# david-strejc/fei

Hardware: AMD Instinct MI355X
Metric: agent tok/s (llama3-8b local decode, 1 agent/GPU) (higher is better)
Workload: dtype bf16; 1 GPU; model=llama3-8b, global_batch=1, seq_len=512, parallelism=dp1 (1 agent per GPU, weak scaling), hip_graph=True, stream_engine=False

## Files before the change

fei_amd/ops/__init__.py:

```python

from __future__ import annotations

import ctypes
import math
import os
from typing import Optional, Tuple

import torch

from fei_amd.ops import reference as ref

_LIB: Optional[ctypes.CDLL] = None
_LIB_ERR: Optional[str] = None
_LIB_PATH = os.path.join(os.path.dirname(os.path.abspath(__file__)),
                         "libfei_kernels.so")

_c = ctypes
_vp, _i, _f, _u64, _l = _c.c_void_p, _c.c_int, _c.c_float, _c.c_ulonglong, _c.c_long


def _try_load() -> None:
    global _LIB, _LIB_ERR
    if _LIB is not None or _LIB_ERR is not None:
        return
    try:
        lib = ctypes.CDLL(_LIB_PATH)
    except OSError as e:
        _LIB_ERR = str(e)
        return
    lib.fei_rmsnorm.argtypes = [_vp, _vp, _vp, _i, _i, _f, _vp]
    lib.fei_add_rmsnorm.argtypes = [_vp, _vp, _vp, _vp, _i, _i, _f, _vp]
    lib.fei_rope_kv_decode.argtypes = [_vp, _vp, _vp, _vp, _vp, _vp, _vp,
                                       _i, _i, _i, _i, _i, _l, _l, _vp]
    lib.fei_rope_kv_prefill.argtypes = [_vp, _vp, _vp, _vp, _vp, _vp, _vp,
                                        _i, _i, _i, _i, _i, _i, _l, _l, _vp]
    lib.fei_attn_decode.argtypes = [_vp, _vp, _vp, _vp, _vp, _vp,
                                    _i, _i, _i, _i, _i, _i, _f, _l,
                                    _vp, _vp, _vp, _l, _vp, _vp, _i, _vp]
    lib.fei_attn_decode_combine.argtypes = [_vp, _vp, _vp, _i, _i, _i, _i, _vp]
    lib.fei_swiglu.argtypes = [_vp, _vp, _l, _i, _vp]
    lib.fei_sample.argtypes = [_vp, _vp, _vp, _vp, _vp, _i, _i, _i, _f, _u64,
                               _i, _vp]
    lib.fei_advance.argtypes = [_vp, _vp, _i, _i, _vp]
    lib.fei_attn_prefill.argtypes = [_vp, _vp, _vp, _vp, _vp, _vp,
                                     _i, _i, _i, _i, _i, _i, _f, _i, _l, _vp]
    lib.fei_mfma_probe.argtypes = [_vp, _vp, _vp, _vp]
    lib.fei_gemv.argtypes = [_vp, _vp, _vp, _i, _i, _i, _i, _vp]
    lib.fei_gemm_m8.argtypes = [_vp, _vp, _vp, _i, _i, _i, _i, _vp]
    lib.fei_attn_decode_fused.argtypes = [_vp, _vp, _vp, _vp, _vp, _vp, _vp,
                                          _vp, _i, _i, _i, _i, _i, _f,
                                          _l, _l, _vp]
    lib.fei_sample_onepass.argtypes = [_vp, _vp, _vp, _vp, _i, _i, _f, _u64,
                                       _i, _vp]
    lib.fei_sample_shard.argtypes = [_vp, _vp, _vp, _i, _i, _i, _f, _u64, _vp]
    lib.fei_sample_filtered.argtypes = [_vp, _vp, _vp, _vp, _vp, _i, _i, _i,
                                        _f, _f, _u64, _i, _vp]
    lib.fei_sample_filtered_rows.argtypes = [_vp, _vp, _vp, _vp, _vp, _vp,
                                             _vp, _vp, _i, _i, _vp]
    lib.fei_sample_filtered_rows.restype = _i
    lib.fei_rope_kv8_decode.argtypes = [_vp, _vp, _vp, _vp, _vp, _vp, _vp,
                                        _vp, _vp, _i, _i, _i, _i, _i, _l, _l,
                                        _vp]
    lib.fei_rope_kv8_prefill.argtypes = [_vp, _vp, _vp, _vp, _vp, _vp, _vp,
                                         _vp, _vp, _i, _i, _i, _i, _i, _i,
                                         _l, _l, _vp]
    lib.fei_attn_decode_kv8.argtypes = [_vp, _vp, _vp, _vp, _vp, _vp, _vp,
                                        _vp, _i, _i, _i, _i, _i, _i, _f, _l,
                                        _vp, _vp, _vp, _l, _vp]
    lib.fei_attn_decode_kv8.restype = _i
    lib.fei_attn_prefill_kv8.argtypes = [_vp, _vp, _vp, _vp, _vp, _vp, _vp,
                                         _i, _i, _i, _i, _i, _i, _f, _l, _vp]
    lib.fei_attn_prefill_kv8.restype = _i
    lib.fei_stream_layer_check.argtypes = [_i, _i, _i, _i, _i]
    lib.fei_stream_layer_check.restype = _i
    lib.fei_stream_layer.argtypes = [_vp, _vp, _vp, _vp, _vp, _vp, _vp, _vp,
                                     _vp, _vp, _vp, _vp, _vp, _vp, _vp, _vp,
                                     _vp, _vp, _vp, _i, _i, _i, _i, _i,
                                     _i, _i, _f, _f, _vp]
    lib.fei_attn_decode_paged.argtypes = [_vp, _vp, _vp, _vp, _vp, _vp, _vp,
                                          _i, _i, _i, _i, _i, _i, _i, _f,
                                          _l, _vp, _vp, _vp, _l, _vp]
    lib.fei_rope_kv_prefill_paged.argtypes = [_vp, _vp, _vp, _vp, _vp, _vp,
                                              _vp, _vp, _i, _i, _i, _i, _i,
                                              _i, _i, _l, _l, _vp]
    lib.fei_rope_kv_prefill_paged.restype = _i
    lib.fei_attn_prefill_paged.argtypes = [_vp, _vp, _vp, _vp, _vp, _vp,
                                           _i, _i, _i, _i, _i, _i, _i, _f,
                                           _l, _vp]
    lib.fei_attn_prefill_paged.restype = _i
    lib.fei_rope_kv8_prefill_paged.argtypes = [
        _vp, _vp, _vp, _vp, _vp, _vp, _vp, _vp, _vp, _vp,
        _i, _i, _i, _i, _i, _i, _i, _l, _l, _vp]
    lib.fei_rope_kv8_prefill_paged.restype = _i
    lib.fei_attn_decode_paged_kv8.argtypes = [
        _vp, _vp, _vp, _vp, _vp, _vp, _vp, _vp, _vp,
        _i, _i, _i, _i, _i, _i, _i, _f, _l, _vp, _vp, _vp, _l, _vp]
    lib.fei_attn_decode_paged_kv8.restype = _i
    lib.fei_attn_prefill_paged_kv8.argtypes = [
        _vp, _vp, _vp, _vp, _vp, _vp, _vp, _vp,
        _i, _i, _i, _i, _i, _i, _i, _f, _l, _vp]
    lib.fei_attn_prefill_paged_kv8.restype = _i
    lib.fei_rope_kv_prefill_paged_ragged.argtypes = [
        _vp, _vp, _vp, _vp, _vp, _vp, _vp, _vp, _vp, _vp,
        _i, _i, _i, _i, _i, _i, _i, _l, _l, _vp]
    lib.fei_rope_kv_prefill_paged_ragged.restype = _i
    lib.fei_attn_prefill_paged_ragged.argtypes = [
        _vp, _vp, _vp, _vp, _vp, _vp, _vp, _vp,
        _i, _i, _i, _i, _i, _i, _i, _i, _f, _l, _vp]
    lib.fei_attn_prefill_paged_ragged.restype = _i
    lib.fei_add_layernorm.argtypes = [_vp, _vp, _vp, _vp, _vp, _i, _i, _f,
                                      _i, _vp]
    lib.fei_gelu.argtypes = [_vp, _vp, _l, _vp]
    lib.fei_gemv_norm_fp8.argtypes = [_vp, _vp, _vp, _vp, _vp, _i, _i, _i,
                                      _f, _vp]
    lib.fei_gemv_res_fp8.argtypes = [_vp, _vp, _vp, _vp, _i, _i, _i, _vp]
    lib.fei_gemv_swiglu_norm_fp8.argtypes = [_vp, _vp, _vp, _vp, _vp, _i, _i,
                                             _i, _f, _vp]
    lib.fei_quant_fp8_rows.argtypes = [_vp, _vp, _vp, _i, _i, _vp]
    lib.fei_gemv_swiglu.argtypes = [_vp, _vp, _vp, _i, _i, _i, _i, _vp]
    lib.fei_prefetch.argtypes = [_vp, _l, _vp, _i, _vp]
    lib.fei_gemv_res.argtypes = [_vp, _vp, _vp, _i, _i, _i, _i, _vp, _vp]
    lib.fei_gemv_norm.argtypes = [_vp, _vp, _vp, _vp, _i, _i, _i, _f, _i, _vp,
                                  _vp]
    lib.fei_gemv_swiglu_norm.argtypes = [_vp, _vp, _vp, _vp, _i, _i, _i, _f,
                                         _i, _vp, _vp]
    for fn in (lib.fei_gemv_addnorm, lib.fei_gemv_swiglu_addnorm):
        fn.argtypes = [_vp, _vp, _vp, _vp, _vp, _vp, _i, _i, _i, _f, _i, _i,
                       _vp]
        fn.restype = _i
    lib.fei_gemv_deep.argtypes = [_vp, _vp, _vp, _i, _i, _i, _i, _vp]
    lib.fei_gemv_deep.restype = _i
    _LIB = lib


def kernels_available() -> bool:
    _try_load()
    return _LIB is not None


def require_lib() -> ctypes.CDLL:
    _try_load()
    if _LIB is None:
        raise RuntimeError(
            "fei_amd HIP kernel library not found at "
            f"{_LIB_PATH} ({_LIB_ERR}). Build it with "
            "`python -m fei_amd.ops.build` — GPU execution refuses to fall "
            "back to eager PyTorch.")
    return _LIB


def _stream() -> int:
    return torch.cuda.current_stream().cuda_stream


def _ptr(t: torch.Tensor) -> int:
    return t.data_ptr()




class QuantKV:

    __slots__ = ("data", "scale")

    def __init__(self, data: torch.Tensor, scale: torch.Tensor):
        assert data.dtype == torch.uint8 and scale.dtype == torch.float32
        assert tuple(scale.shape) == tuple(data.shape[:-1])
        assert data.is_contiguous() and scale.is_contiguous(), \
            "QuantKV needs contiguous data and scale"
        assert data.data_ptr() % 16 == 0, "QuantKV data must be 16 B aligned"
        self.data = data
        self.scale = scale

    @classmethod
    def zeros(cls, shape, device) -> "QuantKV":
        return cls(torch.zeros(shape, dtype=torch.uint8, device=device),
                   torch.ones(shape[:-1], dtype=torch.float32, device=device))

    @property
    def shape(self):
        return self.data.shape

    def dequant(self, length: Optional[int] = None) -> torch.Tensor:
        n = self.data.shape[2] if length is None else length
        return ref.dequant_kv_fp8(self.data[:, :, :n], self.scale[:, :, :n])


def _kv8_pair(k_cache, v_cache) -> bool:
    k8, v8 = isinstance(k_cache, QuantKV), isinstance(v_cache, QuantKV)
    if k8 != v8:
        raise TypeError("k_cache and v_cache must both be QuantKV or both "
                        "be tensors")
    return k8


def _check_gqa(name: str, Hq: int, Hkv: int) -> None:
    if Hkv <= 0 or Hq % Hkv != 0 or Hq // Hkv not in (1, 2, 4, 8):
        raise ValueError(f"{name}: unsupported GQA group Hq={Hq}, Hkv={Hkv} "
                         "(Hq/Hkv must be 1, 2, 4 or 8)")


def _check_vec8(name: str, n: int, what: str = "last dimension") -> None:
    if n % 8 != 0:
        raise ValueError(f"{name}: {what} must be a multiple of 8, got {n}")


def rmsnorm(x: torch.Tensor, weight: torch.Tensor, eps: float = 1e-5,
            out: Optional[torch.Tensor] = None) -> torch.Tensor:
    _check_vec8("rmsnorm", x.shape[-1])
    if x.numel() == 0:
        return torch.empty_like(x) if out is None else out
    if not x.is_cuda:
        return ref.rmsnorm(x, weight, eps)
    lib = require_lib()
    x2 = x.contiguous()
    if out is None:
        out = torch.empty_like(x2)
    rows = x2.numel() // x2.shape[-1]
    lib.fei_rmsnorm(_ptr(out), _ptr(x2), _ptr(weight), rows, x2.shape[-1],
                    eps, _stream())
    return out


def fused_add_rmsnorm(x: torch.Tensor, residual: torch.Tensor,
                      weight: torch.Tensor, eps: float = 1e-5,
                      out: Optional[torch.Tensor] = None
                      ) -> Tuple[torch.Tensor, torch.Tensor]:
    _check_vec8("fused_add_rmsnorm", x.shape[-1])
    if not residual.is_contiguous():
        raise ValueError("fused_add_rmsnorm: residual must be contiguous "
                         "(it is updated in place)")
    if x.numel() == 0:
        return (torch.empty_like(x) if out is None else out), residual
    if not x.is_cuda:
        o, res = ref.fused_add_rmsnorm(x, residual, weight, eps)
        residual.copy_(res)
        return o, residual
    lib = require_lib()
    x2 = x.contiguous()
    if out is None:
        out = torch.empty_like(x2)
    rows = x2.numel() // x2.shape[-1]
    lib.fei_add_rmsnorm(_ptr(out), _ptr(residual), _ptr(x2), _ptr(weight),
                        rows, x2.shape[-1], eps, _stream())
    return out, residual


def rope_kv_decode(q, k, v, k_cache, v_cache, pos, table) -> torch.Tensor:
    kv8 = _kv8_pair(k_cache, v_cache)
    if not q.is_cuda:
        if kv8:
            q_out = ref.rope_kv_decode_fp8(
                q, k, v, k_cache.data, k_cache.scale, v_cache.data,
                v_cache.scale, pos, table)
        else:
            q_out = ref.rope_kv_decode(q, k, v, k_cache, v_cache, pos, table)
        q.copy_(q_out)
        return q
    lib = require_lib()
    B, Hq, D = q.shape
    Hkv = k.shape[1]
    assert q.stride(2) == 1 and q.stride(1) == D, "head rows must be contiguous"
    assert k.stride(1) == D and v.stride(1) == D
    assert k.stride(0) == v.stride(0)
    if kv8:
        assert D in (64, 128), f"fp8 KV append supports D in (64,128), got {D}"
        lib.fei_rope_kv8_decode(_ptr(q), _ptr(k), _ptr(v), _ptr(k_cache.data),
                                _ptr(k_cache.scale), _ptr(v_cache.data),
                                _ptr(v_cache.scale), _ptr(table), _ptr(pos),
                                B, Hq, Hkv, D, k_cache.shape[2],
                                q.stride(0), k.stride(0), _stream())
        return q
    lib.fei_rope_kv_decode(_ptr(q), _ptr(k), _ptr(v), _ptr(k_cache),
                           _ptr(v_cache), _ptr(table), _ptr(pos),
                           B, Hq, Hkv, D, k_cache.shape[2],
                           q.stride(0), k.stride(0), _stream())
    return q


def rope_kv_prefill(q, k, v, k_cache, v_cache, pos0, table) -> torch.Tensor:
    kv8 = _kv8_pair(k_cache, v_cache)
    if not q.is_cuda:
# ... 446 lines not shown
_FUSED_CMB = os.environ.get("FEI_FUSED_CMB", "0") == "1"
_ADDNORM_GEMV = os.environ.get("FEI_ADDNORM_GEMV", "1") == "1"
_GEMV_DEEP = os.environ.get("FEI_GEMV_DEEP", "1") == "1"
_GEMV_DEEP_MAX_WG_PER_CU = float(
    os.environ.get("FEI_GEMV_DEEP_MAX_WG_PER_CU", "8") or 8)
_GEMV_DEEP_MAX_TRIPS = 8
_CU_COUNT: dict = {}


def _gemm_m8_ok(M: int, N: int, K: int) -> bool:
    return 4 <= M <= 8 and K % 1024 == 0 and N % 16 == 0


def _gemv_ok(M: int, K: int) -> bool:
    return M in (1, 2, 4, 8) and K % 8 == 0


def _cu_count(device: torch.device) -> int:
    idx = device.index if device.index is not None else \
        torch.cuda.current_device()
    if idx not in _CU_COUNT:
        _CU_COUNT[idx] = torch.cuda.get_device_properties(
            idx).multi_processor_count
    return _CU_COUNT[idx]


def _gemv_deep_ok(M: int, K: int) -> bool:
    return (M == 1 and K > 0 and K % 8 == 0
            and -(-K // 4096) <= _GEMV_DEEP_MAX_TRIPS)


def _gemv_deep_wins(N: int, K: int, device: torch.device) -> bool:
    return (_GEMV_DEEP and _gemv_deep_ok(1, K)
            and (N + 7) // 8 < _GEMV_DEEP_MAX_WG_PER_CU * _cu_count(device))


def linear_decode(x: torch.Tensor, w: torch.Tensor,
                  out: Optional[torch.Tensor] = None,
                  deep: Optional[bool] = None) -> torch.Tensor:
    M = x.numel() // x.shape[-1]
    K = x.shape[-1]
    N = w.shape[0]
    if not x.is_cuda or not (_gemv_ok(M, K) or _gemm_m8_ok(M, N, K)):
        return torch.nn.functional.linear(x, w)
    lib = require_lib()
    x2 = x.contiguous().view(M, K)
    if out is None:
        out = torch.empty(*x.shape[:-1], N, dtype=x.dtype, device=x.device)
    nt = 1 if (N * K * 2 >= _GEMV_NT_MIN_BYTES) else 0
    if _gemm_m8_ok(M, N, K):
        lib.fei_gemm_m8(_ptr(out), _ptr(x2), _ptr(w), M, N, K, 0,
                        _stream())
        return out
    if deep is None:
        deep = M == 1 and _gemv_deep_wins(N, K, x.device)
    if deep:
        rc = lib.fei_gemv_deep(_ptr(out), _ptr(x2), _ptr(w), M, N, K, nt,
                               _stream())
        if rc != 0:
            raise ValueError(
                f"gemv_deep does not take M={M} N={N} K={K} (code {rc})")
        return out
    lib.fei_gemv(_ptr(out), _ptr(x2), _ptr(w), M, N, K, nt, _stream())
    return out


def gemv_swiglu(x: torch.Tensor, wgu: torch.Tensor,
                out: Optional[torch.Tensor] = None) -> torch.Tensor:
    M = x.numel() // x.shape[-1]
    K = x.shape[-1]
    I = wgu.shape[0] // 2
    if not x.is_cuda:
        return ref.swiglu(torch.nn.functional.linear(x, wgu))
    if not (_gemv_ok(M, K) or _gemm_m8_ok(M, 2 * I, K)):
        return swiglu(torch.nn.functional.linear(x, wgu))
    lib = require_lib()
    x2 = x.contiguous().view(M, K)
    if out is None:
        out = torch.empty(*x.shape[:-1], I, dtype=x.dtype, device=x.device)
    nt = 1 if (2 * I * K * 2 >= _GEMV_NT_MIN_BYTES) else 0
    if _gemm_m8_ok(M, 2 * I, K):
        gu = torch.empty(M, 2 * I, dtype=x.dtype, device=x.device)
        lib.fei_gemm_m8(_ptr(gu), _ptr(x2), _ptr(wgu), M, 2 * I, K, 0,
                        _stream())
        lib.fei_swiglu(_ptr(out), _ptr(gu), M, I, _stream())
        return out
    lib.fei_gemv_swiglu(_ptr(out), _ptr(x2), _ptr(wgu), M, I, K, nt,
                        _stream())
    return out


def gemv_res(x: torch.Tensor, w: torch.Tensor, res: torch.Tensor,
             ssq_out: Optional[torch.Tensor] = None) -> torch.Tensor:
    M = x.numel() // x.shape[-1]
    K = x.shape[-1]
    N = w.shape[0]
    if not x.is_cuda or not _gemv_ok(M, K):
        lin = torch.nn.functional.linear(x, w)
        res.copy_((res.float() + lin.float().view_as(res)).to(res.dtype))
        return res
    lib = require_lib()
    x2 = x.contiguous().view(M, K)
    nt = 1 if (N * K * 2 >= _GEMV_NT_MIN_BYTES) else 0
    lib.fei_gemv_res(_ptr(res), _ptr(x2), _ptr(w), M, N, K, nt,
                     _ptr(ssq_out) if ssq_out is not None else None,
                     _stream())
    return res


def gemv_norm(res: torch.Tensor, wnorm: torch.Tensor, w: torch.Tensor,
              eps: float = 1e-5,
              out: Optional[torch.Tensor] = None,
              ssq: Optional[torch.Tensor] = None) -> torch.Tensor:
    M = res.numel() // res.shape[-1]
    K = res.shape[-1]
    N = w.shape[0]
    if not res.is_cuda or not _gemv_ok(M, K):
        return torch.nn.functional.linear(rmsnorm(res, wnorm, eps), w)
    lib = require_lib()
    r2 = res.contiguous().view(M, K)
    if out is None:
        out = torch.empty(*res.shape[:-1], N, dtype=res.dtype, device=res.device)
    nt = 1 if (N * K * 2 >= _GEMV_NT_MIN_BYTES) else 0
    lib.fei_gemv_norm(_ptr(out), _ptr(r2), _ptr(wnorm), _ptr(w), M, N, K,
                      eps, nt, _ptr(ssq) if ssq is not None else None,
                      _stream())
    return out


def gemv_swiglu_norm(res: torch.Tensor, wnorm: torch.Tensor,
                     wgu: torch.Tensor, eps: float = 1e-5,
                     out: Optional[torch.Tensor] = None,
                     ssq: Optional[torch.Tensor] = None) -> torch.Tensor:
    M = res.numel() // res.shape[-1]
    K = res.shape[-1]
    I = wgu.shape[0] // 2
    if not res.is_cuda or not _gemv_ok(M, K):
        gu = torch.nn.functional.linear(rmsnorm(res, wnorm, eps).float(),
                                        wgu.float())
        return ref.swiglu(gu).to(res.dtype)
    lib = require_lib()
    r2 = res.contiguous().view(M, K)
    if out is None:
        out = torch.empty(*res.shape[:-1], I, dtype=res.dtype, device=res.device)
    nt = 1 if (wgu.shape[0] * K * 2 >= _GEMV_NT_MIN_BYTES) else 0
    lib.fei_gemv_swiglu_norm(_ptr(out), _ptr(r2), _ptr(wnorm), _ptr(wgu),
                             M, I, K, eps, nt,
                             _ptr(ssq) if ssq is not None else None,
                             _stream())
    return out



_ADDNORM_ROW_GROUPS = max(1, int(os.environ.get("FEI_ADDNORM_RG", "2") or 2))
_ADDNORM_ROW_GROUPS_SWIGLU = max(
    1, int(os.environ.get("FEI_ADDNORM_RG_SWIGLU", "2") or 2))


def _addnorm_ok(M: int, K: int) -> bool:
    return M == 1 and _gemv_ok(M, K) and M * K * 2 <= 32 * 1024


def _addnorm_check(name: str, delta, res_in, res_out) -> None:
    if not res_in.is_contiguous() or not res_out.is_contiguous():
        raise ValueError(f"{name}: res_in and res_out must be contiguous")
    if res_in.shape != res_out.shape or res_in.dtype != res_out.dtype:
        raise ValueError(f"{name}: res_in and res_out must match in shape "
                         "and dtype")
    if delta.shape != res_in.shape:
        raise ValueError(f"{name}: delta must have the residual's shape")
    a0, b0 = res_in.data_ptr(), res_out.data_ptr()
    nbytes = res_in.numel() * res_in.element_size()
    if a0 < b0 + nbytes and b0 < a0 + nbytes:
        raise ValueError(f"{name}: res_in and res_out must not share storage "
                         "(the new residual cannot be written in place)")


def gemv_addnorm(delta: torch.Tensor, res_in: torch.Tensor,
                 res_out: torch.Tensor, wnorm: torch.Tensor, w: torch.Tensor,
                 eps: float = 1e-5,
                 out: Optional[torch.Tensor] = None) -> torch.Tensor:
    _addnorm_check("gemv_addnorm", delta, res_in, res_out)
    K = res_in.shape[-1]
    M = res_in.numel() // max(K, 1)
    N = w.shape[0]
    if not res_in.is_cuda or not _addnorm_ok(M, K):
        res_out.copy_(res_in)
        x, _ = fused_add_rmsnorm(delta, res_out, wnorm, eps)
        return linear_decode(x, w, out=out)
    lib = require_lib()
    d2 = delta.contiguous()
    if out is None:
        out = torch.empty(*res_in.shape[:-1], N, dtype=res_in.dtype,
                          device=res_in.device)
    nt = 1 if (N * K * 2 >= _GEMV_NT_MIN_BYTES) else 0
    rc = lib.fei_gemv_addnorm(_ptr(out), _ptr(d2), _ptr(res_in),
                              _ptr(res_out), _ptr(wnorm), _ptr(w), M, N, K,
                              eps, nt, _ADDNORM_ROW_GROUPS, _stream())
    if rc != 0:
        raise RuntimeError(f"fei_gemv_addnorm refused the launch (rc={rc})")
    return out


def gemv_swiglu_addnorm(delta: torch.Tensor, res_in: torch.Tensor,
                        res_out: torch.Tensor, wnorm: torch.Tensor,
                        wgu: torch.Tensor, eps: float = 1e-5,
                        out: Optional[torch.Tensor] = None) -> torch.Tensor:
    _addnorm_check("gemv_swiglu_addnorm", delta, res_in, res_out)
    K = res_in.shape[-1]
    M = res_in.numel() // max(K, 1)
    I = wgu.shape[0] // 2
    if not res_in.is_cuda or not _addnorm_ok(M, K):
        res_out.copy_(res_in)
        x, _ = fused_add_rmsnorm(delta, res_out, wnorm, eps)
        return gemv_swiglu(x, wgu, out=out)
    lib = require_lib()
    d2 = delta.contiguous()
    if out is None:
        out = torch.empty(*res_in.shape[:-1], I, dtype=res_in.dtype,
                          device=res_in.device)
    nt = 1 if (wgu.shape[0] * K * 2 >= _GEMV_NT_MIN_BYTES) else 0
    rc = lib.fei_gemv_swiglu_addnorm(_ptr(out), _ptr(d2), _ptr(res_in),
                                     _ptr(res_out), _ptr(wnorm), _ptr(wgu),
                                     M, I, K, eps, nt,
                                     _ADDNORM_ROW_GROUPS_SWIGLU, _stream())
    if rc != 0:
        raise RuntimeError(
            f"fei_gemv_swiglu_addnorm refused the launch (rc={rc})")
    return out


def prefetch(w: torch.Tensor, max_bytes: int, sink: torch.Tensor,
             n_blocks: int = 512, stream=None) -> None:
    if not w.is_cuda:
        return
    lib = require_lib()
    bytes_ = min(max_bytes, w.numel() * w.element_size())
    sp = stream if stream is not None else _stream()
    lib.fei_prefetch(_ptr(w), bytes_, _ptr(sink), n_blocks, sp)


def attn_decode_paged(q, k_pool, v_pool, block_table, pos, splits: int = 32,
                      scale: Optional[float] = None,
                      workspace: Optional[Tuple[torch.Tensor, torch.Tensor]] = None,
                      out: Optional[torch.Tensor] = None,
                      k: Optional[torch.Tensor] = None,
                      v: Optional[torch.Tensor] = None,
                      table: Optional[torch.Tensor] = None) -> torch.Tensor:
    if _kv8_pair(k_pool, v_pool):
        return _attn_decode_paged_kv8(q, k_pool, v_pool, block_table, pos,
                                      splits, scale, workspace, out, k, v,
                                      table)
    B, Hq, D = q.shape
    n_blocks, Hkv, BS, _ = k_pool.shape
    assert BS & (BS - 1) == 0, "block size must be a power of two"
    bs_log = BS.bit_length() - 1
    scale = scale if scale is not None else 1.0 / math.sqrt(D)
    if not q.is_cuda:
        if table is not None:
            q = ref.apply_rope(q, pos.long(), table).to(q.dtype)
            k_r = ref.apply_rope(k, pos.long(), table).to(k.dtype)
            for b in range(B):
                p = int(pos[b])
                blk = int(block_table[b, p >> bs_log])
                k_pool[blk, :, p & (BS - 1), :] = k_r[b]
                v_pool[blk, :, p & (BS - 1), :] = v[b]
        max_len = block_table.shape[1] * BS
        kc = torch.zeros(B, Hkv, max_len, D, dtype=k_pool.dtype)
        vc = torch.zeros_like(kc)
        for b in range(B):
            for j, blk in enumerate(block_table[b].tolist()):
                if blk < 0:
                    continue
                kc[b, :, j * BS:(j + 1) * BS] = k_pool[blk]
                vc[b, :, j * BS:(j + 1) * BS] = v_pool[blk]
        return ref.attn_decode(q, kc, vc, pos + 1, scale)
    lib = require_lib()
    _check_gqa("attn_decode_paged", Hq, Hkv)
    if workspace is None:
        part_o = torch.empty(B, Hq, splits, D, dtype=torch.float32, device=q.device)
        part_ml = torch.empty(B, Hq, splits, 2, dtype=torch.float32, device=q.device)
    else:
        part_o, part_ml = workspace
        assert part_o.shape[2] == splits and part_ml.shape[2] == splits
    if out is None:
        out = torch.empty_like(q)
    assert q.stride(2) == 1 and q.stride(1) == D
    assert D in (64, 128), f"paged attention supports D in (64,128), got {D}"
    assert splits <= 64
    if table is not None:
        assert k is not None and v is not None
        assert k.stride(1) == D and k.stride(0) == v.stride(0)
        kin, vin, cs, kv_bs = _ptr(k), _ptr(v), _ptr(table), k.stride(0)
    else:
        kin = vin = cs = None
        kv_bs = 0
    lib.fei_attn_decode_paged(_ptr(q), _ptr(k_pool), _ptr(v_pool),
                              _ptr(block_table), _ptr(part_o), _ptr(part_ml),
                              _ptr(pos), B, Hq, Hkv, D, bs_log,
                              block_table.shape[1], splits, scale,
                              q.stride(0), kin, vin, cs, kv_bs, _stream())
    lib.fei_attn_decode_combine(_ptr(out), _ptr(part_o), _ptr(part_ml),
                                B, Hq, D, splits, _stream())
    return out



def _paged_check(name: str, q, k_pool, block_table, pos0) -> Tuple[int, int]:
    B, S, Hq, D = q.shape
    Hkv, BS = k_pool.shape[1], k_pool.shape[2]
    if Hkv <= 0 or Hq % Hkv != 0:
        raise ValueError(f"{name}: Hq={Hq} is not a multiple of Hkv={Hkv}")
    if BS <= 0 or BS & (BS - 1):
        raise ValueError(f"{name}: block size must be a power of two, "
                         f"got {BS}")
    if q.is_cuda and D not in (64, 128):
        raise ValueError(f"{name} supports D in (64,128), got {D}")
    if block_table.dim() != 2 or block_table.shape[0] != B or \
            block_table.dtype != torch.int32:
        raise ValueError(f"{name}: block_table must be int32 [B, max_blocks]")
    if not pos0.is_cuda and B > 0 and \
            block_table.shape[1] * BS < int(pos0.max()) + S:
        raise ValueError(
            f"{name}: block_table covers {block_table.shape[1] * BS} rows, "
            f"the prefill reaches row {int(pos0.max()) + S}")
    return Hkv, BS


def _gather_pool(pool: torch.Tensor, block_table: torch.Tensor,
                 n_rows) -> torch.Tensor:
    _, Hkv, BS, D = pool.shape
    B = block_table.shape[0]
    out = pool.new_zeros(B, Hkv, max(max(n_rows), 1), D)
    for b in range(B):
        for j in range(0, n_rows[b], BS):
            n = min(BS, n_rows[b] - j)
            out[b, :, j:j + n] = pool[int(block_table[b, j // BS]), :, :n]
    return out


def _gather_pool_kv8(pool: QuantKV, block_table: torch.Tensor,
                     n_rows) -> torch.Tensor:
    data = _gather_pool(pool.data, block_table, n_rows)
    scale = _gather_pool(pool.scale.unsqueeze(-1), block_table,
                         n_rows).squeeze(-1)
    return ref.dequant_kv_fp8(data, scale)


def _scatter_pool_kv8(pool: QuantKV, block_table: torch.Tensor, b: int,
                      p: int, codes: torch.Tensor, scales: torch.Tensor):
    BS = pool.shape[2]
    blk = int(block_table[b, p // BS])
    pool.data[blk, :, p % BS, :] = codes
    pool.scale[blk, :, p % BS] = scales


def _attn_decode_paged_kv8(q, k_pool, v_pool, block_table, pos, splits, scale,
                           workspace, out, k, v, table) -> torch.Tensor:
    B, Hq, D = q.shape
    _, Hkv, BS, _ = k_pool.shape
    name = "attn_decode_paged (fp8)"
    if BS <= 0 or BS & (BS - 1):
        raise ValueError(f"{name}: block size must be a power of two, "
                         f"got {BS}")
    scale = scale if scale is not None else 1.0 / math.sqrt(D)
    if not q.is_cuda:
        if table is not None:
            q = ref.apply_rope(q, pos.long(), table)
            kq, ks = ref.quant_kv_fp8(ref.apply_rope(k, pos.long(), table))
            vq, vs = ref.quant_kv_fp8(v)
            for b in range(B):
                p = int(pos[b])
                _scatter_pool_kv8(k_pool, block_table, b, p, kq[b], ks[b])
                _scatter_pool_kv8(v_pool, block_table, b, p, vq[b], vs[b])
        n_rows = [int(pos[b]) + 1 for b in range(B)]
        return ref.attn_decode(q, _gather_pool_kv8(k_pool, block_table, n_rows),
                               _gather_pool_kv8(v_pool, block_table, n_rows),
                               pos + 1, scale)
    lib = require_lib()
    _check_gqa(name, Hq, Hkv)
    if D not in (64, 128):
# ... 425 lines not shown
```

fei_amd/ops/csrc/gemv_addnorm.hip:

```cpp
#include "fei_common.h"

namespace {

constexpr int PRE = 8;
constexpr int PRO = 2;

template <bool NT>
__device__ __forceinline__ s16x8 ldw(const s16x8* p) {
  return NT ? __builtin_nontemporal_load(p) : *p;
}

template <bool NT>
__device__ __forceinline__ void preload_row(s16x8 (&wv)[PRE],
                                            const s16x8* __restrict__ wrow,
                                            int nv, int lane) {
#pragma unroll
  for (int u = 0; u < PRE; ++u)
    wv[u] = ldw<NT>(&wrow[min(lane + u * 64, nv - 1)]);
}

struct AddnormIn { s16x8 d[PRO], h[PRO], w[PRO]; };

__device__ __forceinline__ void addnorm_issue(AddnormIn& in,
                                              const s16x8* __restrict__ dr,
// ... 48 lines not shown
    ss = i < nv ? s2 : ss;
    if (ho && i < nv) ho[i] = nr[u];
  }
  for (int i = tid + PRO * 256; i < nv; i += 256) {
    s16x8 n;
    ss = addnorm_sumsq8(hr[i], dr[i], n, ss);
    xs[i] = n;
    if (ho) ho[i] = n;
  }
  ss = block_reduce_sum(ss, red);
  const float inv = rsqrtf(ss / (float)K + eps);
#pragma unroll
  for (int u = 0; u < PRO; ++u) {
    const int i = tid + u * 256;
    const s16x8 o = addnorm_scale8(nr[u], in.w[u], inv);
    if (i < nv) xs[i] = o;
  }
  for (int i = tid + PRO * 256; i < nv; i += 256)
    xs[i] = addnorm_scale8(xs[i], wr[i], inv);
  __syncthreads();
}

template <bool NT>
__device__ __forceinline__ void dot_rows(float& acc0, float& acc1,
                                         const s16x8 (&wv0)[PRE],
                                         const s16x8 (&wv1)[PRE],
                                         const s16x8* __restrict__ wrow0,
                                         const s16x8* __restrict__ wrow1,
                                         const s16x8* xs, int nv, int lane) {
#pragma unroll
  for (int u = 0; u < PRE; ++u) {
    const int i = lane + u * 64;
    const s16x8 xv = xs[min(i, nv - 1)];
    const float d0 = dot8_bf16(xv, wv0[u]);
    const float d1 = dot8_bf16(xv, wv1[u]);
    acc0 = i < nv ? acc0 + d0 : acc0;
    acc1 = i < nv ? acc1 + d1 : acc1;
    __builtin_amdgcn_sched_barrier(0);
  }
  for (int i = lane + PRE * 64; i < nv; i += 64) {
    const s16x8 a = ldw<NT>(&wrow0[i]);
    const s16x8 b = ldw<NT>(&wrow1[i]);
    const s16x8 xv = xs[i];
    acc0 += dot8_bf16(xv, a);
    acc1 += dot8_bf16(xv, b);
  }
}

#define ADDNORM_LDS(K) ((size_t)(K) * 2 + 4 * sizeof(float))

template <int M, bool NT>
__global__ void __launch_bounds__(256)
k_gemv_addnorm(u16* __restrict__ out, const u16* __restrict__ delta,
               const u16* __restrict__ h_in, u16* __restrict__ h_out,
               const u16* __restrict__ wn, const u16* __restrict__ w,
               int N, int K, float eps, int rg) {
  static_assert(M == 1, "the add+norm prologue is batch-1 only");
  extern __shared__ s16x8 lds_x[];
  s16x8* xs = lds_x;
  float* red = (float*)(lds_x + (K >> 3));
  const int tid = threadIdx.x;
  const int lane = tid & 63;
  const int wid = tid >> 6;
  const int nv = K >> 3;
  int n0 = blockIdx.x * rg * 8 + wid * 2;

  bool active = n0 < N;
  bool two = (n0 + 1) < N;
  const s16x8* wrow0 = (const s16x8*)(w + (long)(active ? n0 : 0) * K);
  const s16x8* wrow1 =
      (const s16x8*)(w + (long)(active ? n0 + (two ? 1 : 0) : 0) * K);

  const s16x8* dr = (const s16x8*)delta;
  const s16x8* hr = (const s16x8*)h_in;
  const s16x8* wr = (const s16x8*)wn;
  AddnormIn in;
  addnorm_issue(in, dr, hr, wr, nv, tid);
  s16x8 wv0[PRE], wv1[PRE];
  preload_row<NT>(wv0, wrow0, nv, lane);
  preload_row<NT>(wv1, wrow1, nv, lane);
  addnorm_finish(in, xs, red, dr, hr, wr,
                 blockIdx.x == 0 ? (s16x8*)h_out : nullptr, nv, K, eps, tid);

  for (int g = 0;;) {
    float acc0 = 0.f, acc1 = 0.f;
    dot_rows<NT>(acc0, acc1, wv0, wv1, wrow0, wrow1, xs, nv, lane);
    const float v0 = wave_reduce_sum(acc0);
    const float v1 = wave_reduce_sum(acc1);
    if (lane == 0 && active) {
      out[n0] = f2bf(v0);
      if (two) out[n0 + 1] = f2bf(v1);
    }
    if (++g >= rg) break;
    n0 += 8;
    active = n0 < N;
    two = (n0 + 1) < N;
    wrow0 = (const s16x8*)(w + (long)(active ? n0 : 0) * K);
    wrow1 = (const s16x8*)(w + (long)(active ? n0 + (two ? 1 : 0) : 0) * K);
    preload_row<NT>(wv0, wrow0, nv, lane);
    preload_row<NT>(wv1, wrow1, nv, lane);
  }
}

template <int M, bool NT>
__global__ void __launch_bounds__(256)
k_gemv_swiglu_addnorm(u16* __restrict__ out, const u16* __restrict__ delta,
                      const u16* __restrict__ h_in, u16* __restrict__ h_out,
                      const u16* __restrict__ wn, const u16* __restrict__ w,
                      int N, int K, float eps, int rg) {
  static_assert(M == 1, "the add+norm prologue is batch-1 only");
  extern __shared__ s16x8 lds_x[];
  s16x8* xs = lds_x;
  float* red = (float*)(lds_x + (K >> 3));
  const int tid = threadIdx.x;
  const int lane = tid & 63;
  const int wid = tid >> 6;
  const int nv = K >> 3;
  int n = blockIdx.x * rg * 4 + wid;

  bool active = n < N;
  const s16x8* grow = (const s16x8*)(w + (long)(active ? n : 0) * K);
  const s16x8* urow = (const s16x8*)(w + (long)((active ? n : 0) + N) * K);

  const s16x8* dr = (const s16x8*)delta;
  const s16x8* hr = (const s16x8*)h_in;
  const s16x8* wr = (const s16x8*)wn;
  AddnormIn in;
  addnorm_issue(in, dr, hr, wr, nv, tid);
  s16x8 gv[PRE], uv[PRE];
  preload_row<NT>(gv, grow, nv, lane);
  preload_row<NT>(uv, urow, nv, lane);
  addnorm_finish(in, xs, red, dr, hr, wr,
                 blockIdx.x == 0 ? (s16x8*)h_out : nullptr, nv, K, eps, tid);

  for (int g = 0;;) {
    float accg = 0.f, accu = 0.f;
    dot_rows<NT>(accg, accu, gv, uv, grow, urow, xs, nv, lane);
    const float gs = wave_reduce_sum(accg);
    const float us = wave_reduce_sum(accu);
    if (lane == 0 && active) {
      const float silu = gs / (1.f + __expf(-gs));
      out[n] = f2bf(silu * us);
    }
    if (++g >= rg) break;
    n += 4;
    active = n < N;
    grow = (const s16x8*)(w + (long)(active ? n : 0) * K);
    urow = (const s16x8*)(w + (long)((active ? n : 0) + N) * K);
    preload_row<NT>(gv, grow, nv, lane);
    preload_row<NT>(uv, urow, nv, lane);
  }
}

}

extern "C" {

int fei_gemv_addnorm(void* out, const void* delta, const void* h_in,
                     void* h_out, const void* wn, const void* w, int M, int N,
                     int K, float eps, int nontemporal, int row_groups,
                     hipStream_t stream) {
  if (M != 1) return -1;
  if (K <= 0 || K % 8 != 0 || (size_t)K * 2 > 32 * 1024 || N < 1) return -2;
  if (h_in == h_out) return -3;
  const int rg = row_groups < 1 ? 1 : row_groups;
  const int groups = (N + 7) / 8;
  dim3 grid((groups + rg - 1) / rg);
#define LA(NTV) hipLaunchKernelGGL((k_gemv_addnorm<1, NTV>), grid, dim3(256), \
    ADDNORM_LDS(K), stream, (u16*)out, (const u16*)delta, (const u16*)h_in, \
    (u16*)h_out, (const u16*)wn, (const u16*)w, N, K, eps, rg)
  if (nontemporal) LA(true); else LA(false);
#undef LA
  return 0;
}

int fei_gemv_swiglu_addnorm(void* out, const void* delta, const void* h_in,
                            void* h_out, const void* wn, const void* w, int M,
                            int N, int K, float eps, int nontemporal,
                            int row_groups, hipStream_t stream) {
  if (M != 1) return -1;
  if (K <= 0 || K % 8 != 0 || (size_t)K * 2 > 32 * 1024 || N < 1) return -2;
  if (h_in == h_out) return -3;
  const int rg = row_groups < 1 ? 1 : row_groups;
  const int groups = (N + 3) / 4;
  dim3 grid((groups + rg - 1) / rg);
#define LA(NTV) hipLaunchKernelGGL((k_gemv_swiglu_addnorm<1, NTV>), grid, \
    dim3(256), ADDNORM_LDS(K), stream, (u16*)out, (const u16*)delta, \
    (const u16*)h_in, (u16*)h_out, (const u16*)wn, (const u16*)w, N, K, eps, rg)
  if (nontemporal) LA(true); else LA(false);
#undef LA
  return 0;
}

}
```

Measured before the change: 329.7 tok/s.

## Add ring-pipelined addnorm GEMV kernels with compile-time trip counts

Adds new fused add-RMSNorm+GEMV and SwiGLU variants in which each wave keeps two weight rows in registers and refills them for the next strided row group while it computes the current dot products. Loads for the next trip overlap compute, so the drain between row groups goes away. The kernels use grid-stride scheduling with a compile-time trip count and an occupancy-based auto planner. By default the new path is on, and the SwiGLU row-group count rises to 5. This cuts redundant per-block norm recomputation but risks register pressure and lower occupancy.

```diff
diff --git a/fei_amd/ops/__init__.py b/fei_amd/ops/__init__.py
--- a/fei_amd/ops/__init__.py
+++ b/fei_amd/ops/__init__.py
@@ -128,6 +128,14 @@
         fn.argtypes = [_vp, _vp, _vp, _vp, _vp, _vp, _i, _i, _i, _f, _i, _i,
                        _vp]
         fn.restype = _i
+    for fn in (lib.fei_gemv_addnorm_ring, lib.fei_gemv_swiglu_addnorm_ring):
+        fn.argtypes = [_vp, _vp, _vp, _vp, _vp, _vp, _i, _i, _i, _f, _i, _i,
+                       _i, _vp]
+        fn.restype = _i
+    lib.fei_gemv_addnorm_ring_slots.argtypes = [_i, _i, _i, _i]
+    lib.fei_gemv_addnorm_ring_slots.restype = _i
+    lib.fei_gemv_addnorm_ring_max_trips.argtypes = []
+    lib.fei_gemv_addnorm_ring_max_trips.restype = _i
     lib.fei_gemv_deep.argtypes = [_vp, _vp, _vp, _i, _i, _i, _i, _vp]
     lib.fei_gemv_deep.restype = _i
     _LIB = lib
@@ -880,9 +888,88 @@
 
 
 
-_ADDNORM_ROW_GROUPS = max(1, int(os.environ.get("FEI_ADDNORM_RG", "2") or 2))
-_ADDNORM_ROW_GROUPS_SWIGLU = max(
-    1, int(os.environ.get("FEI_ADDNORM_RG_SWIGLU", "2") or 2))
+_ADDNORM_RING = os.environ.get("FEI_ADDNORM_RING", "1") != "0"
+
+_ADDNORM_DRAIN_RG = 2
+_ADDNORM_RG_DEFAULT = 2
+_ADDNORM_RG_SWIGLU_DEFAULT = 5 if _ADDNORM_RING else _ADDNORM_DRAIN_RG
+_ADDNORM_ROW_GROUPS = max(0, int(
+    os.environ.get("FEI_ADDNORM_RG", "") or _ADDNORM_RG_DEFAULT))
+_ADDNORM_ROW_GROUPS_SWIGLU = max(0, int(
+    os.environ.get("FEI_ADDNORM_RG_SWIGLU", "") or _ADDNORM_RG_SWIGLU_DEFAULT))
+
+_ADDNORM_RING_MAX_K = 4096
+_ADDNORM_RING_MAX_TRIPS = 8
+
+
+def _addnorm_plan(groups: int, slots: int,
+                  max_trips: int = _ADDNORM_RING_MAX_TRIPS) -> Tuple[int, int]:
+    if groups < 1 or slots < 1:
+        raise ValueError("groups and slots must be positive")
+    grid = min(groups, slots)
+    trips = -(-groups // grid)
+    if trips > max_trips:
+        trips = max_trips
+        grid = -(-groups // trips)
+    return grid, trips
+
+
+def _addnorm_fixed_plan(groups: int, rg: int) -> Tuple[int, int]:
+    return -(-groups // rg), rg
+
+
+_ADDNORM_SLOTS: dict = {}
+_ADDNORM_PLANS: dict = {}
+
+
+def _addnorm_slots(swiglu: bool, nt: int, trips: int, K: int) -> int:
+    key = (bool(swiglu), int(nt), int(trips), int(K),
+           torch.cuda.current_device())
+    slots = _ADDNORM_SLOTS.get(key)
+    if slots is None:
+        slots = require_lib().fei_gemv_addnorm_ring_slots(
+            int(swiglu), int(nt), int(trips), int(K))
+        if slots < 1:
+            raise RuntimeError(
+                f"fei_gemv_addnorm_ring_slots failed (rc={slots})")
+        _ADDNORM_SLOTS[key] = slots
+    return slots
+
+
+def _addnorm_auto_plan(swiglu: bool, nt: int, K: int,
+                       groups: int) -> Tuple[int, int]:
+    key = (bool(swiglu), int(nt), int(K), int(groups),
+           torch.cuda.current_device())
+    plan = _ADDNORM_PLANS.get(key)
+    if plan is None:
+        for t in range(1, _ADDNORM_RING_MAX_TRIPS + 1):
+            plan = _addnorm_plan(groups, _addnorm_slots(swiglu, nt, t, K))
+            if plan[1] <= t:
+                break
+        _ADDNORM_PLANS[key] = plan
+    return plan
+
+
+def _addnorm_launch(swiglu: bool, rg: int, out, delta, res_in, res_out, wnorm,
+                    w, M: int, N: int, K: int, eps: float, nt: int) -> None:
+    lib = require_lib()
+    name = "fei_gemv_swiglu_addnorm" if swiglu else "fei_gemv_addnorm"
+    ptrs = (_ptr(out), _ptr(delta), _ptr(res_in), _ptr(res_out), _ptr(wnorm),
+            _ptr(w))
+    if (_ADDNORM_RING and K <= _ADDNORM_RING_MAX_K
+            and rg <= _ADDNORM_RING_MAX_TRIPS):
+        groups = -(-N // (4 if swiglu else 8))
+        grid, trips = (_addnorm_fixed_plan(groups, rg) if rg >= 1 else
+                       _addnorm_auto_plan(swiglu, nt, K, groups))
+        name += "_ring"
+        rc = getattr(lib, name)(*ptrs, M, N, K, eps, nt, grid, trips,
+                                _stream())
+    else:
+        rc = getattr(lib, name)(*ptrs, M, N, K, eps, nt,
+                                rg if rg >= 1 else _ADDNORM_DRAIN_RG,
+                                _stream())
+    if rc != 0:
+        raise RuntimeError(f"{name} refused the launch (rc={rc})")
 
 
 def _addnorm_ok(M: int, K: int) -> bool:
@@ -922,11 +1009,8 @@
         out = torch.empty(*res_in.shape[:-1], N, dtype=res_in.dtype,
                           device=res_in.device)
     nt = 1 if (N * K * 2 >= _GEMV_NT_MIN_BYTES) else 0
-    rc = lib.fei_gemv_addnorm(_ptr(out), _ptr(d2), _ptr(res_in),
-                              _ptr(res_out), _ptr(wnorm), _ptr(w), M, N, K,
-                              eps, nt, _ADDNORM_ROW_GROUPS, _stream())
-    if rc != 0:
-        raise RuntimeError(f"fei_gemv_addnorm refused the launch (rc={rc})")
+    _addnorm_launch(False, _ADDNORM_ROW_GROUPS, out, d2, res_in, res_out,
+                    wnorm, w, M, N, K, eps, nt)
     return out
 
 
@@ -948,13 +1032,8 @@
         out = torch.empty(*res_in.shape[:-1], I, dtype=res_in.dtype,
                           device=res_in.device)
     nt = 1 if (wgu.shape[0] * K * 2 >= _GEMV_NT_MIN_BYTES) else 0
-    rc = lib.fei_gemv_swiglu_addnorm(_ptr(out), _ptr(d2), _ptr(res_in),
-                                     _ptr(res_out), _ptr(wnorm), _ptr(wgu),
-                                     M, I, K, eps, nt,
-                                     _ADDNORM_ROW_GROUPS_SWIGLU, _stream())
-    if rc != 0:
-        raise RuntimeError(
-            f"fei_gemv_swiglu_addnorm refused the launch (rc={rc})")
+    _addnorm_launch(True, _ADDNORM_ROW_GROUPS_SWIGLU, out, d2, res_in,
+                    res_out, wnorm, wgu, M, I, K, eps, nt)
     return out
 
 
diff --git a/fei_amd/ops/csrc/gemv_addnorm.hip b/fei_amd/ops/csrc/gemv_addnorm.hip
--- a/fei_amd/ops/csrc/gemv_addnorm.hip
+++ b/fei_amd/ops/csrc/gemv_addnorm.hip
@@ -224,9 +224,247 @@
   }
 }
 
+
+constexpr int RING_MAX_TRIPS = 8;
+
+template <bool NT>
+__device__ __forceinline__ void preload_rows(s16x8 (&wv0)[PRE],
+                                             s16x8 (&wv1)[PRE],
+                                             const s16x8* __restrict__ wrow0,
+                                             const s16x8* __restrict__ wrow1,
+                                             int nv, int lane) {
+#pragma unroll
+  for (int u = 0; u < PRE; ++u) {
+    const int j = min(lane + u * 64, nv - 1);
+    wv0[u] = ldw<NT>(&wrow0[j]);
+    wv1[u] = ldw<NT>(&wrow1[j]);
+  }
+}
+
+template <bool NT, bool REFILL>
+__device__ __forceinline__ void dot_rows_ring(float& acc0, float& acc1,
+                                              s16x8 (&wv0)[PRE],
+                                              s16x8 (&wv1)[PRE],
+                                              const s16x8* __restrict__ next0,
+                                              const s16x8* __restrict__ next1,
+                                              const s16x8* xs, int nv,
+                                              int lane) {
+#pragma unroll
+  for (int u = 0; u < PRE; ++u) {
+    const int i = lane + u * 64;
+    const int j = min(i, nv - 1);
+    const s16x8 xv = xs[j];
+    const float d0 = dot8_bf16(xv, wv0[u]);
+    const float d1 = dot8_bf16(xv, wv1[u]);
+    acc0 = i < nv ? acc0 + d0 : acc0;
+    acc1 = i < nv ? acc1 + d1 : acc1;
+    if (REFILL) {
+      int jr = j;
+      asm volatile("" : "+v"(jr), "+v"(acc0), "+v"(acc1));
+      wv0[u] = ldw<NT>(&next0[jr]);
+      wv1[u] = ldw<NT>(&next1[jr]);
+    }
+    __builtin_amdgcn_sched_barrier(0);
+  }
+}
+
+template <bool NT, int G>
+__global__ void __launch_bounds__(256)
+k_gemv_addnorm_ring(u16* __restrict__ out, const u16* __restrict__ delta,
+                    const u16* __restrict__ h_in, u16* __restrict__ h_out,
+                    const u16* __restrict__ wn, const u16* __restrict__ w,
+                    int N, int K, float eps) {
+  extern __shared__ s16x8 lds_x[];
+  s16x8* xs = lds_x;
+  float* red = (float*)(lds_x + (K >> 3));
+  const int tid = threadIdx.x;
+  const int lane = tid & 63;
+  const int wid = tid >> 6;
+  const int nv = K >> 3;
+  const long stride = (long)gridDim.x * 8;
+  long n0 = (long)blockIdx.x * 8 + wid * 2;
+
+  bool active = n0 < N;
+  bool two = (n0 + 1) < N;
+  const s16x8* wrow0 = (const s16x8*)(w + (active ? n0 : 0) * K);
+  const s16x8* wrow1 = (const s16x8*)(w + (active ? n0 + (two ? 1 : 0) : 0) * K);
+
+  const s16x8* dr = (const s16x8*)delta;
+  const s16x8* hr = (const s16x8*)h_in;
+  const s16x8* wr = (const s16x8*)wn;
+  AddnormIn in;
+  addnorm_issue(in, dr, hr, wr, nv, tid);
+  s16x8 wv0[PRE], wv1[PRE];
+  preload_rows<NT>(wv0, wv1, wrow0, wrow1, nv, lane);
+  addnorm_finish(in, xs, red, dr, hr, wr,
+                 blockIdx.x == 0 ? (s16x8*)h_out : nullptr, nv, K, eps, tid);
+
+#pragma unroll
+  for (int g = 0; g < G; ++g) {
+    float acc0 = 0.f, acc1 = 0.f;
+    const long nn = n0 + stride;
+    const bool nactive = nn < N;
+    const bool ntwo = (nn + 1) < N;
+    if (g + 1 < G) {
+      wrow0 = (const s16x8*)(w + (nactive ? nn : 0) * K);
+      wrow1 = (const s16x8*)(w + (nactive ? nn + (ntwo ? 1 : 0) : 0) * K);
+      dot_rows_ring<NT, true>(acc0, acc1, wv0, wv1, wrow0, wrow1, xs, nv,
+                              lane);
+    } else {
+      dot_rows_ring<NT, false>(acc0, acc1, wv0, wv1, wrow0, wrow1, xs, nv,
+                               lane);
+    }
+    const float v0 = wave_reduce_sum(acc0);
+    const float v1 = wave_reduce_sum(acc1);
+    if (lane == 0 && active) {
+      out[n0] = f2bf(v0);
+      if (two) out[n0 + 1] = f2bf(v1);
+    }
+    n0 = nn;
+    active = nactive;
+    two = ntwo;
+  }
+}
+
+template <bool NT, int G>
+__global__ void __launch_bounds__(256)
+k_gemv_swiglu_addnorm_ring(u16* __restrict__ out,
+                           const u16* __restrict__ delta,
+                           const u16* __restrict__ h_in,
+                           u16* __restrict__ h_out,
+                           const u16* __restrict__ wn,
+                           const u16* __restrict__ w, int N, int K,
+                           float eps) {
+  extern __shared__ s16x8 lds_x[];
+  s16x8* xs = lds_x;
+  float* red = (float*)(lds_x + (K >> 3));
+  const int tid = threadIdx.x;
+  const int lane = tid & 63;
+  const int wid = tid >> 6;
+  const int nv = K >> 3;
+  const long stride = (long)gridDim.x * 4;
+  long n = (long)blockIdx.x * 4 + wid;
+
+  bool active = n < N;
+  const long up = (long)N * nv;
+  const s16x8* grow = (const s16x8*)(w + (active ? n : 0) * K);
+  const s16x8* urow = grow + up;
+
+  const s16x8* dr = (const s16x8*)delta;
+  const s16x8* hr = (const s16x8*)h_in;
+  const s16x8* wr = (const s16x8*)wn;
+  AddnormIn in;
+  addnorm_issue(in, dr, hr, wr, nv, tid);
+  s16x8 gv[PRE], uv[PRE];
+  preload_rows<NT>(gv, uv, grow, urow, nv, lane);
+  addnorm_finish(in, xs, red, dr, hr, wr,
+                 blockIdx.x == 0 ? (s16x8*)h_out : nullptr, nv, K, eps, tid);
+
+#pragma unroll
+  for (int g = 0; g < G; ++g) {
+    float accg = 0.f, accu = 0.f;
+    const long nn = n + stride;
+    const bool nactive = nn < N;
+    if (g + 1 < G) {
+      grow = (const s16x8*)(w + (nactive ? nn : 0) * K);
+      urow = grow + up;
+      dot_rows_ring<NT, true>(accg, accu, gv, uv, grow, urow, xs, nv, lane);
+    } else {
+      dot_rows_ring<NT, false>(accg, accu, gv, uv, grow, urow, xs, nv, lane);
+    }
+    const float gs = wave_reduce_sum(accg);
+    const float us = wave_reduce_sum(accu);
+    if (lane == 0 && active) {
+      const float silu = gs / (1.f + __expf(-gs));
+      out[n] = f2bf(silu * us);
+    }
+    n = nn;
+    active = nactive;
+  }
+}
+
+template <int G>
+const void* ring_instance(bool swiglu, bool nt) {
+  if (swiglu)
+    return nt ? (const void*)k_gemv_swiglu_addnorm_ring<true, G>
+              : (const void*)k_gemv_swiglu_addnorm_ring<false, G>;
+  return nt ? (const void*)k_gemv_addnorm_ring<true, G>
+            : (const void*)k_gemv_addnorm_ring<false, G>;
+}
+
+const void* ring_kernel(bool swiglu, bool nt, int trips) {
+  switch (trips) {
+    case 1: return ring_instance<1>(swiglu, nt);
+    case 2: return ring_instance<2>(swiglu, nt);
+    case 3: return ring_instance<3>(swiglu, nt);
+    case 4: return ring_instance<4>(swiglu, nt);
+    case 5: return ring_instance<5>(swiglu, nt);
+    case 6: return ring_instance<6>(swiglu, nt);
+    case 7: return ring_instance<7>(swiglu, nt);
+    case 8: return ring_instance<8>(swiglu, nt);
+    default: return nullptr;
+  }
+}
+
+bool ring_shape_ok(int K) {
+  return K > 0 && K % 8 == 0 && (K >> 3) <= PRE * 64;
+}
+
+int ring_launch(bool swiglu, void* out, const void* delta, const void* h_in,
+                void* h_out, const void* wn, const void* w, int M, int N,
+                int K, float eps, int nontemporal, int grid, int trips,
+                hipStream_t stream) {
+  if (M != 1) return -1;
+  if (!ring_shape_ok(K) || N < 1) return -2;
+  if (h_in == h_out) return -3;
+  const long groups = swiglu ? ((long)N + 3) / 4 : ((long)N + 7) / 8;
+  const void* fn = ring_kernel(swiglu, nontemporal != 0, trips);
+  if (!fn || grid < 1 || (long)grid * trips < groups) return -4;
+  void* args[] = {&out, &delta, &h_in, &h_out, &wn, &w, &N, &K, &eps};
+  if (hipLaunchKernel(fn, dim3(grid), dim3(256), args, ADDNORM_LDS(K),
+                      stream) != hipSuccess)
+    return -5;
+  return 0;
+}
+
 }
 
 extern "C" {
+
+int fei_gemv_addnorm_ring_max_trips(void) { return RING_MAX_TRIPS; }
+
+int fei_gemv_addnorm_ring_slots(int swiglu, int nontemporal, int trips,
+                                int K) {
+  if (!ring_shape_ok(K)) return -2;
+  const void* fn = ring_kernel(swiglu != 0, nontemporal != 0, trips);
+  if (!fn) return -4;
+  int dev = 0, cus = 0, per_cu = 0;
+  if (hipGetDevice(&dev) != hipSuccess ||
+      hipDeviceGetAttribute(&cus, hipDeviceAttributeMultiprocessorCount,
+                            dev) != hipSuccess ||
+      hipOccupancyMaxActiveBlocksPerMultiprocessor(
+          &per_cu, fn, 256, ADDNORM_LDS(K)) != hipSuccess)
+    return -5;
+  if (per_cu < 1 || cus < 1) return -5;
+  return per_cu * cus;
+}
+
+int fei_gemv_addnorm_ring(void* out, const void* delta, const void* h_in,
+                          void* h_out, const void* wn, const void* w, int M,
+                          int N, int K, float eps, int nontemporal, int grid,
+                          int trips, hipStream_t stream) {
+  return ring_launch(false, out, delta, h_in, h_out, wn, w, M, N, K, eps,
+                     nontemporal, grid, trips, stream);
+}
+
+int fei_gemv_swiglu_addnorm_ring(void* out, const void* delta,
+                                 const void* h_in, void* h_out,
+                                 const void* wn, const void* w, int M, int N,
+                                 int K, float eps, int nontemporal, int grid,
+                                 int trips, hipStream_t stream) {
+  return ring_launch(true, out, delta, h_in, h_out, wn, w, M, N, K, eps,
+                     nontemporal, grid, trips, stream);
+}
 
 int fei_gemv_addnorm(void* out, const void* delta, const void* h_in,
                      void* h_out, const void* wn, const void* w, int M, int N,
```

Measured after the change: 337.7 tok/s (median of 6 runs). +2.5%, better.
